# thomwiggers/m4ri-rust

Measured on AMD Instinct MI355X. Metric: gf2_matmul_bit_ops_per_sec_n65536, higher is better.
Workload: dtype u64

## Files before the change

m4ri-rust_amd/csrc/gf2_kernels.h:

```cpp
#pragma once
#include <hip/hip_runtime.h>
#include <stdint.h>

struct gf2k_mul_args {
  const uint64_t *A;
  const uint64_t *B;
  uint64_t *C;
  long long lda, ldb, ldc;
  long long sA, sB, sC;
  int m, l, n;
  int tiles_m, tiles_n;
  int ksplit;
  int kwords;
  int batch;
  int accumulate;
  const uint32_t *Bp;
  long long sBp;
  int bp_nc;
  uint64_t *P;
  long long ldp, sP;
  int a_packed;
  int n_rem, nseg;
  long long p_words;
  int n_full, seg_slabs, tile_slabs;
// ... 8 lines not shown
  int scan;
  int lastword;
  unsigned long long pcmask;
  int cur_row[64];
  int cntP, cnt2;
  int err;
};
enum { GF2K_ELIM_BLOCK_PIVOTS = 2048 };

extern "C" {
hipError_t gf2k_elim_begin_block(gf2k_elim_state *st, hipStream_t s);
hipError_t gf2k_elim_step(uint64_t *A, long long lda, int m, long long c0w, int sw, int j, uint64_t colmask, int full,
                          uint64_t *U, long long ldu, int uw, gf2k_elim_state *st, int *pivcols, uint64_t *ptab,
                          unsigned char *rowflag, int *blkpiv, uint64_t colmask_next, int lookahead, hipStream_t s);
hipError_t gf2k_elim_end_block(uint64_t *A, long long lda, long long aw, long long c0w, uint64_t *U, long long ldu, int uw,
                               gf2k_elim_state *st, unsigned char *rowflag, const int *blkpiv, int *moves, uint64_t *tmp,
                               long long tld, long long w_right, hipStream_t s);
hipError_t gf2k_elim_small(uint64_t *A, long long lda, int m, int ncols, int limit, int full, int *rank_out, int *pivcols,
                           hipStream_t s);
enum {
  GF2K_ELIM_BATCH_WAVE1 = 0,
  GF2K_ELIM_BATCH_WAVE2 = 1,
  GF2K_ELIM_BATCH_WAVE4 = 2,
  GF2K_ELIM_BATCH_WAVE8 = 3,
  GF2K_ELIM_BATCH_WAVE16 = 4,
  GF2K_ELIM_BATCH_WAVE_INV = 5,
  GF2K_ELIM_BATCH_LDS = 6,
  GF2K_ELIM_BATCH_LDS_INV = 7,
  GF2K_ELIM_BATCH_VARIANTS = 8
};
enum { GF2K_ELIM_BATCH_WAVE_THREADS = 256 };
hipError_t gf2k_elim_batch(const uint64_t *S, long long lds_, uint64_t *D, long long ldd, int m, int ncols, int limit, int full,
                           int inverse, long long batch, int *ranks, int *pivcols, int *singular, hipStream_t s);
hipError_t gf2k_set_diag(uint64_t *M, long long ld, int n, long long col0, hipStream_t s);
hipError_t gf2k_scatter_rows(uint64_t *X, long long ldx, const uint64_t *R, long long ldr, int words, const int *pivcols,
                             int rank, hipStream_t s);
hipError_t gf2k_any_nonzero(const uint64_t *M, long long ld, int row_lo, int rows, int cols, int *flag, hipStream_t s);
int gf2k_m4rm_rows_per_tile(int cfg);
long long gf2k_m4rm_streamk_words(int cfg, int nseg);
int gf2k_m4rm_cols_per_tile(int cfg);
hipError_t gf2k_packA(uint64_t *dst, long long wp, const uint64_t *src, long long lds_, int m, int w, hipStream_t stream);
hipError_t gf2k_m4rm(gf2k_mul_args a, int cfg, hipStream_t stream);
#ifdef GF2K_DEV_VARIANTS
hipError_t gf2k_dbg_sec(unsigned long long *out8);
int gf2k_packB_chunks(int l);
hipError_t gf2k_packB(uint32_t *Bp, long long bpStride, const uint64_t *B, long long ldb, long long bStride, int l, int n,
                      int batch, hipStream_t stream);
#endif
hipError_t gf2k_rowparity(const uint64_t *A, long long lda, const uint64_t *Bt, long long ldbt, uint64_t *C, long long ldc,
                          int m, int l, int n, int accumulate, hipStream_t stream);
hipError_t gf2k_narrow(const uint64_t *A, long long lda, const uint64_t *B, long long ldb, uint64_t *C, long long ldc,
                       int m, int l, int n, int accumulate, hipStream_t stream);
hipError_t gf2k_widevec(const uint64_t *A, long long lda, const uint64_t *Bt, long long ldbt, uint64_t *C, long long ldc,
                        int m, int l, int n, int accumulate, int jshift, hipStream_t stream);
hipError_t gf2k_tallskinny(const uint64_t *A, long long lda, const uint64_t *B, long long ldb, uint64_t *C, long long ldc,
                           int m, int l, int n, int accumulate, hipStream_t stream);
hipError_t gf2k_tallskinny_side(const uint64_t *A, long long lda, const uint64_t *B, long long ldb, uint64_t *C, long long ldc, int m,
                                int l, int n, uint64_t *side, long long side_ld, hipStream_t stream);
hipError_t gf2k_tallskinny_long(const uint64_t *A, long long lda, const uint64_t *B, long long ldb, uint64_t *C, long long ldc,
                                int m, int l, int n, int accumulate, hipStream_t stream);
hipError_t gf2k_va(const uint64_t *A, long long lda, const uint64_t *B, long long ldb, uint64_t *C, long long ldc, int m,
                   int l, int n, hipStream_t stream);
hipError_t gf2k_xor2d(uint64_t *C, long long ldc, const uint64_t *A, long long lda, const uint64_t *B, long long ldb,
                      int rows, int words, hipStream_t stream);
hipError_t gf2k_padcopy(uint64_t *dst, long long ldd, int drows, int dwords, const uint64_t *src, long long lds_, int srows,
                        int scols, hipStream_t stream);
hipError_t gf2k_copy_block(uint64_t *D, long long ldd, long long dr, long long dc, const uint64_t *S, long long lds_, long long sr,
                           long long sc, int nrows, int ncols, int accumulate, int zero_tail, hipStream_t stream);
hipError_t gf2k_fill_random(uint64_t *M, long long ld, int rows, int cols, uint64_t seed, long long row0, long long fullw,
                            long long colw0, hipStream_t stream);
hipError_t gf2k_diff(const uint64_t *A, long long lda, const uint64_t *B, long long ldb, int rows, int cols, int *diff,
                     hipStream_t stream);
hipError_t gf2k_transpose(uint64_t *D, long long ldd, const uint64_t *S, long long lds_, int rows, int cols,
                          hipStream_t stream);
hipError_t gf2k_strassen_split(uint64_t *dst, long long ldd, long long dstStride, const uint64_t *src, long long lds_,
                               long long srcStride, int h, int w, int side, int batch, hipStream_t stream);
hipError_t gf2k_strassen_split2(uint64_t *dst, long long ldd, long long dstStride, const uint64_t *src, long long lds_,
                                long long srcStride, int h, int w, int side, int batch, hipStream_t stream);
hipError_t gf2k_strassen_split3(uint64_t *dst, long long ldd, long long dstStride, const uint64_t *const *src0,
                                const uint64_t *const *src1, int groups, long long lds_, long long srcStride, int h, int w, int side,
                                int batch, hipStream_t stream);
hipError_t gf2k_strassen_merge3(uint64_t *dst, long long ldd, long long dstStride, const uint64_t *src, long long lds_,
                                long long srcStride, int h, int w, int accumulate, int groups, int batch, hipStream_t stream);
hipError_t gf2k_strassen_merge2(uint64_t *dst, long long ldd, long long dstStride, const uint64_t *src, long long lds_,
                                long long srcStride, int h, int w, int accumulate, int batch, hipStream_t stream);
hipError_t gf2k_strassen_merge(uint64_t *dst, long long ldd, long long dstStride, const uint64_t *src, long long lds_,
                               long long srcStride, int h, int w, int accumulate, int batch, hipStream_t stream);
}

void gf2k_note_launch(const void *kernel);
#undef hipLaunchKernelGGL
#define hipLaunchKernelGGL(kernelName, ...)                        \
  do {                                                             \
    gf2k_note_launch(reinterpret_cast<const void *>(kernelName));  \
    hipLaunchKernelGGLInternal((kernelName), __VA_ARGS__);         \
  } while (0)
```

m4ri-rust_amd/csrc/gf2_kernels.hip:

```cpp
#include <hip/hip_runtime.h>
#include <stdint.h>
#include <stdio.h>
#include <stdlib.h>
#include <algorithm>
#include <mutex>
#include <set>
#include <type_traits>
#include <utility>
#include "gf2_kernels.h"
#include "gf2_variants.h"

typedef uint64_t u64;
typedef uint32_t u32;

#ifdef GF2K_DEV_VARIANTS
#define GF2K_DEV_ENV(name, dflt) (getenv(name) ? atoi(getenv(name)) : (dflt))
__device__ unsigned long long *gf2k_clock_stamps;
extern "C" hipError_t gf2k_dev_set_clock_stamps(unsigned long long *p) {
  return hipMemcpyToSymbol(HIP_SYMBOL(gf2k_clock_stamps), &p, sizeof(p));
}
#else
#define GF2K_DEV_ENV(name, dflt) (dflt)
#endif

// ... 1964 lines not shown
      constexpr int a1 = kStrassenSupp[SIDE][q1][0], b1 = kStrassenSupp[SIDE][q1][1];
      u64 y[16];
      static_for<16>([&](auto J) {
        constexpr int j = decltype(J)::value;
        y[j] = b1 >= 0 ? (x[a1 * 16 + j] ^ x[(b1 < 0 ? 0 : b1) * 16 + j]) : x[a1 * 16 + j];
      });
      static_for<7>([&](auto Q2) {
        constexpr int q2 = decltype(Q2)::value;
        constexpr int a2 = kStrassenSupp[SIDE][q2][0], b2 = kStrassenSupp[SIDE][q2][1];
        u64 z[4];
        static_for<4>([&](auto J) {
          constexpr int j = decltype(J)::value;
          z[j] = b2 >= 0 ? (y[a2 * 4 + j] ^ y[(b2 < 0 ? 0 : b2) * 4 + j]) : y[a2 * 4 + j];
        });
        static_for<7>([&](auto Q3) {
          constexpr int q3 = decltype(Q3)::value;
          constexpr int a3 = kStrassenSupp[SIDE][q3][0], b3 = kStrassenSupp[SIDE][q3][1];
          const u64 o = b3 >= 0 ? (z[a3] ^ z[b3 < 0 ? 0 : b3]) : z[a3];
          if (NT) __builtin_nontemporal_store(o, &Y[(long long)(49 * q1 + 7 * q2 + q3) * dstStride + at]);
          else Y[(long long)(49 * q1 + 7 * q2 + q3) * dstStride + at] = o;
        });
      });
    });
  }
}

__device__ constexpr int kStrassenFoldTo[7][2] = {{0, 3}, {2, 3}, {1, 3}, {0, 2}, {0, 1}, {3, -1}, {0, -1}};

template <bool NT>
__global__ __launch_bounds__(256) void gf2_strassen_merge3_kernel(u64 *__restrict__ dst, long long ldd, long long dstStride,
                                                                  const u64 *__restrict__ src, long long lds_,
                                                                  long long srcStride, int h, int w, int accumulate) {
  const long long parent = (long long)blockIdx.z * gridDim.y + blockIdx.y;
  const u64 *M = src + parent * 343 * srcStride;
  u64 *Cq = dst + parent * dstStride;
  const long long total = (long long)h * w;
  for (long long idx = (long long)blockIdx.x * blockDim.x + threadIdx.x; idx < total; idx += (long long)gridDim.x * blockDim.x) {
    const int r = (int)(idx / w), c = (int)(idx % w);
    const u64 *Mp = M + (long long)r * lds_ + c;
    u64 z[64];
    static_for<64>([&](auto K) { z[decltype(K)::value] = 0; });
#pragma unroll 1
    for (int q1 = 0; q1 < 7; ++q1) {
      u64 y[16];
      static_for<16>([&](auto J) { y[decltype(J)::value] = 0; });
      const u64 *Mq = Mp + (long long)(49 * q1) * srcStride;
      static_for<7>([&](auto Q2) {
        constexpr int q2 = decltype(Q2)::value;
        u64 m[7];
        static_for<7>([&](auto Q3) {
          constexpr int q3 = decltype(Q3)::value;
          m[q3] = NT ? __builtin_nontemporal_load(&Mq[(long long)(7 * q2 + q3) * srcStride]) : Mq[(long long)(7 * q2 + q3) * srcStride];
        });
        const u64 f[4] = {m[0] ^ m[3] ^ m[4] ^ m[6], m[2] ^ m[4], m[1] ^ m[3], m[0] ^ m[1] ^ m[2] ^ m[5]};
        constexpr int t0 = kStrassenFoldTo[q2][0], t1 = kStrassenFoldTo[q2][1];
        static_for<4>([&](auto J) {
          constexpr int j = decltype(J)::value;
          y[t0 * 4 + j] ^= f[j];
          if (t1 >= 0) y[(t1 < 0 ? 0 : t1) * 4 + j] ^= f[j];
        });
      });
      const int u0 = kStrassenFoldTo[q1][0], u1 = kStrassenFoldTo[q1][1];
      static_for<4>([&](auto U) {
        constexpr int u = decltype(U)::value;
        const u64 mask = (u == u0 || u == u1) ? ~0ull : 0ull;
        static_for<16>([&](auto J) {
          constexpr int j = decltype(J)::value;
          z[u * 16 + j] ^= y[j] & mask;
        });
      });
    }
    static_for<64>([&](auto K) {
      constexpr int k = decltype(K)::value;
      constexpr int R = 4 * ((k >> 5) & 1) + 2 * ((k >> 3) & 1) + ((k >> 1) & 1);
      constexpr int Cc = 4 * ((k >> 4) & 1) + 2 * ((k >> 2) & 1) + (k & 1);
      u64 *pd = Cq + (long long)(r + R * h) * ldd + (long long)Cc * w + c;
      u64 v = z[k];
      if (accumulate) v ^= *pd;
      if (NT) __builtin_nontemporal_store(v, pd);
      else *pd = v;
    });
  }
}


static inline int grid_for(long long total, int block = 256, int cap = 256 * 8) {
  long long g = (total + block - 1) / block;
  if (g < 1) g = 1;
  if (g > cap) g = cap;
  return (int)g;
}

static int cfg_v8_rg(int cfg) { return gf2_variant_of(cfg).v8_rg; }
static int cfg_v9_rg(int cfg) { return gf2_variant_of(cfg).v9_rg; }
extern "C" int gf2k_m4rm_rows_per_tile(int cfg) { return gf2_variant_of(cfg).rows; }
extern "C" int gf2k_m4rm_cols_per_tile(int cfg) { return gf2_variant_of(cfg).cols; }
extern "C" long long gf2k_m4rm_streamk_words(int cfg, int nseg) { return gf2_streamk_words(gf2_variant_of(cfg), nseg); }

static hipError_t lds_limit_once(const void *kernel, int bytes) {
  static std::mutex mu;
  static std::set<std::pair<const void *, int>> done;
  int dev = 0;
  if (hipGetDevice(&dev) != hipSuccess) dev = 0;
  std::lock_guard<std::mutex> lk(mu);
  if (done.count({kernel, dev})) return hipSuccess;
  const hipError_t e = hipFuncSetAttribute(kernel, hipFuncAttributeMaxDynamicSharedMemorySize, bytes);
  if (e == hipSuccess) done.insert({kernel, dev});
  return e;
}

template <typename K>
static hipError_t launch_tile_kernel(K kernel, int threads, const gf2k_mul_args &a, long long nwg, hipStream_t stream) {
  hipError_t e = lds_limit_once(reinterpret_cast<const void *>(kernel), kLdsBytes);
  if (e != hipSuccess) {
    fprintf(stderr, "gf2k: hipFuncSetAttribute failed: %s\n", hipGetErrorString(e));
    return e;
  }
  hipLaunchKernelGGL(kernel, dim3((unsigned)nwg), dim3(threads), kLdsBytes, stream, a);
  e = hipGetLastError();
  if (e != hipSuccess) fprintf(stderr, "gf2k: tile kernel launch failed: %s\n", hipGetErrorString(e));
  return e;
}

static hipError_t launch_v8(gf2k_mul_args a, int cfg, int RG, hipStream_t stream) {
  const bool v9 = cfg_v9_rg(cfg) != 0;
  const int R = 512 * RG, TC = v9 ? 128 : 512;
  a.tiles_m = (a.m + R - 1) / R;
  a.tiles_n = (a.n + TC - 1) / TC;
  const long long T = (long long)a.tiles_m * a.tiles_n * a.batch;
  if (T > 0x7fffff00LL) return hipErrorInvalidValue;
  const int nw32 = (a.l + 31) / 32, Q = v9 ? (nw32 + 3) / 4 : (nw32 + 1) / 2;
  a.tile_slabs = Q;
  if (a.ksplit > 1 && a.n_rem <= 0) a.n_rem = (int)T, a.nseg = (int)std::min<long long>(T * a.ksplit, 1 << 20);
  a.ksplit = 1;
  a.kwords = 0;
#ifdef GF2K_DEV_VARIANTS
  static const int v8_flags = getenv("GF2K_V8_FLAGS") ? atoi(getenv("GF2K_V8_FLAGS")) : 0;
  a.kwords = v8_flags;
#endif
  long long n_rem = a.P && Q > 0 ? std::min<long long>(std::max(a.n_rem, 0), T) : 0;
  gf2_streamk_cut cut = gf2_streamk_cut_of(T, Q, n_rem, a.nseg);
  if (cut.nseg > 0x7fffff00LL - T || gf2_streamk_words(gf2_variant_of(cfg), cut.nseg) > a.p_words) cut = {0, 0, 0};
  n_rem = cut.n_rem;
  const int nseg = (int)cut.nseg, seg = (int)cut.seg;
  a.n_rem = (int)n_rem;
  a.nseg = nseg;
  a.seg_slabs = seg;
  a.n_full = (int)(T - n_rem);
  a.sP = (long long)R * (v9 ? 2 : 8);
  const long long nwg = (long long)a.n_full + nseg;
  if (nwg <= 0) return hipSuccess;
  hipError_t e = hipErrorInvalidValue;
#define GF2K_V8G(RGv, Gv)                                                                              \
  e = a.a_packed ? launch_tile_kernel(&gf2_m4rm_kernel_v8<RGv, Gv, 1>, 512, a, nwg, stream)            \
                 : launch_tile_kernel(&gf2_m4rm_kernel_v8<RGv, Gv, 0>, 512, a, nwg, stream)
#define GF2K_V8(RGv) GF2K_V8G(RGv, 2)
#define GF2K_V9(RGv)                                                                                   \
  e = a.a_packed ? launch_tile_kernel(&gf2_m4rm_kernel_v9<RGv, 2, 1>, 512, a, nwg, stream)             \
                 : launch_tile_kernel(&gf2_m4rm_kernel_v9<RGv, 2, 0>, 512, a, nwg, stream)
#ifdef GF2K_DEV_VARIANTS
  if (v9) {
    switch (RG) {
      case 8: GF2K_V9(8); break;
      case 4: GF2K_V9(4); break;
      default: GF2K_V9(2); break;
    }
// ... 545 lines not shown
    const long long ntp = (long long)((tx_n + stw - 1) / stw) * ((ty_n + 7) / 8) * (stw * 8);
    if (ntp > 0x7fffffffLL) return hipErrorInvalidValue;
    static const int tgrid = GF2K_DEV_ENV("M4RI_HIP_TRANSPOSE_GRID", (1 << 20));
    dim3 grid((unsigned)std::min<long long>(ntp, tgrid)), block(512);
    hipLaunchKernelGGL(gf2_transpose512_kernel, grid, block, 0, stream, D, ldd, S, lds_, rows, cols, (int)ntp, tflags);
    return hipGetLastError();
  }
  dim3 grid((sw + 3) / 4, rb), block(256);
  hipLaunchKernelGGL(gf2_transpose_kernel, grid, block, 0, stream, D, ldd, S, lds_, rows, cols);
  return hipGetLastError();
}

extern "C" hipError_t gf2k_strassen_split(u64 *dst, long long ldd, long long dstStride, const u64 *src, long long lds_,
                                          long long srcStride, int h, int w, int side, int batch, hipStream_t stream) {
  if (h <= 0 || w <= 0 || batch <= 0) return hipSuccess;
  const long long total = (long long)h * (w / 2);
  int gx = grid_for(total, 256, (4096 + batch - 1) / batch);
  hipLaunchKernelGGL(gf2_strassen_split_kernel, dim3(gx, 1, batch), dim3(256), 0, stream, dst, ldd, dstStride, src, lds_,
                     srcStride, h, w, side);
  return hipGetLastError();
}

extern "C" hipError_t gf2k_strassen_split2(u64 *dst, long long ldd, long long dstStride, const u64 *src, long long lds_,
                                           long long srcStride, int h, int w, int side, int batch, hipStream_t stream) {
  if (h <= 0 || w <= 0 || batch <= 0) return hipSuccess;
  const long long total = (long long)h * (w / 2);
  int gx = grid_for(total, 256, (4096 + batch - 1) / batch);
  hipLaunchKernelGGL(gf2_strassen_split2_kernel, dim3(gx, 1, batch), dim3(256), 0, stream, dst, ldd, dstStride, src, lds_,
                     srcStride, h, w, side);
  return hipGetLastError();
}

extern "C" hipError_t gf2k_strassen_split3(u64 *dst, long long ldd, long long dstStride, const u64 *const *src0,
                                           const u64 *const *src1, int groups, long long lds_, long long srcStride, int h, int w,
                                           int side, int batch, hipStream_t stream) {
  if (h <= 0 || w <= 0 || batch <= 0 || groups <= 0) return hipSuccess;
  if (groups > 7 || (side == 2 && (h & 63))) return hipErrorInvalidValue;
  gf2k_split3_srcs srcs{};
  for (int g = 0; g < groups; ++g) {
    srcs.a[g] = src0[g];
    srcs.b[g] = src1 ? src1[g] : nullptr;
  }
  const long long total = (long long)h * w;
  static const int cap = GF2K_DEV_ENV("M4RI_HIP_PASS_GRID", 8192);
  const int gx = grid_for(total, 256, (cap + batch * groups - 1) / (batch * groups));
  const dim3 grid(gx * groups, 1, batch);
  static const int nt = GF2K_DEV_ENV("M4RI_HIP_PASS_NT", 1);
#ifdef GF2K_DEV_VARIANTS
  if (!nt && side == 2)
    hipLaunchKernelGGL((gf2_strassen_split3_kernel<0, true>), grid, dim3(256), 0, stream, dst, ldd, dstStride, srcs, lds_, srcStride, h, w, gx);
  else if (!nt && side == 1)
    hipLaunchKernelGGL((gf2_strassen_split3_kernel<1, false>), grid, dim3(256), 0, stream, dst, ldd, dstStride, srcs, lds_, srcStride, h, w, gx);
  else
#endif
  if (side == 2)
    hipLaunchKernelGGL((gf2_strassen_split3_kernel<0, true, true>), grid, dim3(256), 0, stream, dst, ldd, dstStride, srcs, lds_, srcStride, h, w, gx);
  else if (side == 0)
    hipLaunchKernelGGL((gf2_strassen_split3_kernel<0, false>), grid, dim3(256), 0, stream, dst, ldd, dstStride, srcs, lds_, srcStride, h, w, gx);
  else
    hipLaunchKernelGGL((gf2_strassen_split3_kernel<1, false, true>), grid, dim3(256), 0, stream, dst, ldd, dstStride, srcs, lds_, srcStride, h, w, gx);
  (void)nt;
  return hipGetLastError();
}

extern "C" hipError_t gf2k_strassen_merge3(u64 *dst, long long ldd, long long dstStride, const u64 *src, long long lds_,
                                           long long srcStride, int h, int w, int accumulate, int groups, int batch,
                                           hipStream_t stream) {
  if (h <= 0 || w <= 0 || batch <= 0 || groups <= 0) return hipSuccess;
  const long long total = (long long)h * w;
  const int gx = grid_for(total, 256, (8192 + batch * groups - 1) / (batch * groups));
  static const int ntl = GF2K_DEV_ENV("M4RI_HIP_PASS_NTL", 1);
#ifdef GF2K_DEV_VARIANTS
  if (!ntl)
    hipLaunchKernelGGL(gf2_strassen_merge3_kernel<false>, dim3(gx, groups, batch), dim3(256), 0, stream, dst, ldd, dstStride, src, lds_,
                       srcStride, h, w, accumulate);
  else
#endif
    hipLaunchKernelGGL(gf2_strassen_merge3_kernel<true>, dim3(gx, groups, batch), dim3(256), 0, stream, dst, ldd, dstStride, src, lds_,
                       srcStride, h, w, accumulate);
  (void)ntl;
  return hipGetLastError();
}

extern "C" hipError_t gf2k_strassen_merge2(u64 *dst, long long ldd, long long dstStride, const u64 *src, long long lds_,
                                           long long srcStride, int h, int w, int accumulate, int batch,
                                           hipStream_t stream) {
  if (h <= 0 || w <= 0 || batch <= 0) return hipSuccess;
  const long long total = (long long)h * (w / 2);
  int gx = grid_for(total, 256, (4096 + batch - 1) / batch);
  hipLaunchKernelGGL(gf2_strassen_merge2_kernel, dim3(gx, 1, batch), dim3(256), 0, stream, dst, ldd, dstStride, src, lds_,
                     srcStride, h, w, accumulate);
  return hipGetLastError();
}

extern "C" hipError_t gf2k_strassen_merge(u64 *dst, long long ldd, long long dstStride, const u64 *src, long long lds_,
                                          long long srcStride, int h, int w, int accumulate, int batch,
                                          hipStream_t stream) {
  if (h <= 0 || w <= 0 || batch <= 0) return hipSuccess;
  const long long total = (long long)h * (w / 2);
  int gx = grid_for(total, 256, (4096 + batch - 1) / batch);
  hipLaunchKernelGGL(gf2_strassen_merge_kernel, dim3(gx, 1, batch), dim3(256), 0, stream, dst, ldd, dstStride, src, lds_,
                     srcStride, h, w, accumulate);
  return hipGetLastError();
}
```

m4ri-rust_amd/csrc/mul_dev_host.cpp:

```cpp
#include <algorithm>
#include <cstdint>
#include <vector>

#include "dev_args.h"
#include "gf2_kernels.h"
#include "mul_plan.h"

typedef uint64_t u64;

static int sync_if(bool sync_free, hipStream_t s) {
  return sync_free && hipStreamSynchronize(s) != hipSuccess ? gf2_fail_hip(hipGetLastError(), "hipStreamSynchronize") : 0;
}
static int launch_m4rm(gf2k_mul_args a, int cfg, hipStream_t s) {
  HIP_TRY(gf2k_m4rm(a, cfg, s));
  return 0;
}

static int apply_tile_plan(gf2k_mul_args &a, const TilePlan &tp, hipStream_t s) {
  a.ksplit = 1;
  a.n_rem = a.nseg = 0;
  a.P = nullptr;
  a.p_words = 0;
  const size_t want = tp.scratch();
  if (want == 0) return 0;
// ... 162 lines not shown
  const std::vector<PlanStep> plan = strassen_plan(L);
  u64 *Aop[7], *Bop[7], *Pop[7];
  auto at = [&](size_t off) { return off == StrassenArena::none ? nullptr : static_cast<u64 *>(ws) + off; };
  for (int i = 0; i < 7; ++i) Aop[i] = at(arena.a[i]), Bop[i] = at(arena.b[i]), Pop[i] = at(arena.p[i]);
  bool a_packed = false;
  const TilePlan leaf = leaf_plan(m, l, n, L, &a_packed);

  auto split_step = [&](const PlanStep &st, int prev, int i, int side, bool pack) -> int {
    const bool isA = side == 0;
    const int rows_prev = (isA ? m : l) >> prev, rows_i = (isA ? m : l) >> i;
    const int words_prev = ((isA ? l : n) >> prev) / 64, words_i = ((isA ? l : n) >> i) / 64;
    const int batch = (int)pow7(prev);
    const gf2_dmat *top = isA ? A : B;
    const u64 *src = prev ? (isA ? Aop[prev] : Bop[prev]) : top->data;
    const long long lds_ = prev ? (long long)words_prev : top->ld;
    const long long srcStride = prev ? (long long)rows_prev * lds_ : 0;
    u64 *dst = isA ? Aop[i] : Bop[i];
    const long long dstStride = (long long)rows_i * words_i;
    const int kside = pack ? 2 : side;
    if (st.k == 1) return (int)gf2k_strassen_split(dst, words_i, dstStride, src, lds_, srcStride, rows_i, words_i, kside, batch, s);
    if (st.k == 2) return (int)gf2k_strassen_split2(dst, words_i, dstStride, src, lds_, srcStride, rows_i, words_i, kside, batch, s);
    const u64 *s0[7], *s1[7];
    int groups = 1;
    s0[0] = src;
    s1[0] = nullptr;
    if (st.virt) {
      groups = 7;
      const long long hq = rows_prev / 2, wq = words_prev / 2;
      auto quad = [&](int q) { return src + (long long)(q >> 1) * hq * lds_ + (long long)(q & 1) * wq; };
      for (int g = 0; g < 7; ++g) {
        s0[g] = quad(kSupp[side][g][0]);
        s1[g] = kSupp[side][g][1] >= 0 ? quad(kSupp[side][g][1]) : nullptr;
      }
    }
    return (int)gf2k_strassen_split3(dst, words_i, dstStride, s0, s1, groups, lds_, srcStride, rows_i, words_i, kside, batch, s);
  };

  auto run = [&]() -> int {
    int prev = 0;
    for (size_t k = 0; k < plan.size(); ++k) {
      const int i = prev + plan[k].levels();
      const bool last = k + 1 == plan.size();
      HIP_TRY((hipError_t)split_step(plan[k], prev, i, 0, last && a_packed));
      HIP_TRY((hipError_t)split_step(plan[k], prev, i, 1, false));
      prev = i;
    }
    {
      const int mL = m >> L, lL = l >> L, nL = n >> L;
      gf2k_mul_args a{};
      a.lda = lL / 64;
      a.ldb = nL / 64;
      a.ldc = nL / 64;
      a.sA = (long long)mL * a.lda;
      a.sB = (long long)lL * a.ldb;
      a.sC = (long long)mL * a.ldc;
      a.A = Aop[L];
      a.B = Bop[L];
      a.C = Pop[L];
      a.m = mL;
      a.l = lL;
      a.n = nL;
      a.batch = (int)pow7(L);
      a.accumulate = 0;
      a.a_packed = a_packed ? 1 : 0;
      if (int r = launch_planned(a, leaf, s)) return r;
    }
    int i = L;
    for (int k = (int)plan.size() - 1; k >= 0; --k) {
      const PlanStep &st = plan[k];
      const int up = i - st.levels();
      const int mi = m >> i, wi = (n >> i) / 64, batch = (int)pow7(up);
      u64 *dst = up ? Pop[up] : C->data;
      const long long ldd = up ? (long long)((n >> up) / 64) : C->ld;
      const long long strD = up ? (long long)(m >> up) * ldd : 0;
      const int acc = up ? 0 : accumulate;
      const long long dP = (long long)mi * wi;
      if (st.k == 1) {
        HIP_TRY(gf2k_strassen_merge(dst, ldd, strD, Pop[i], wi, dP, mi, wi, acc, batch, s));
      } else if (st.k == 2) {
        HIP_TRY(gf2k_strassen_merge2(dst, ldd, strD, Pop[i], wi, dP, mi, wi, acc, batch, s));
      } else if (!st.virt) {
        HIP_TRY(gf2k_strassen_merge3(dst, ldd, strD, Pop[i], wi, dP, mi, wi, acc, 1, batch, s));
      } else {
        const int m1 = m >> (up + 1), w1 = (n >> (up + 1)) / 64;
        HIP_TRY(gf2k_strassen_merge3(Pop[up + 1], w1, (long long)m1 * w1, Pop[i], wi, dP, mi, wi, 0, 7, batch, s));
        HIP_TRY(gf2k_strassen_merge(dst, ldd, strD, Pop[up + 1], w1, (long long)m1 * w1, m1, w1, acc, batch, s));
      }
      i = up;
    }
    return 0;
  };
  const int rc = run();
  return rc ? rc : sync_if(sync_free, s);
}

static int cap_levels_by_memory(int m, int l, int n, int L, hipStream_t s, size_t extra_bytes = 0) {
  if (L <= 0) return L;
  const size_t avail = gf2_dev_arena_limit(s);
  while (L > 0 && strassen_arena(m, l, n, L).words * sizeof(u64) + extra_bytes > avail) --L;
  return L;
}

std::mutex gf2_enqueue_mu;

static int mul_strassen_padded(gf2_dmat *C, const gf2_dmat *A, const gf2_dmat *B, int accumulate, const MulPlan &pp, hipStream_t s) {
  const int m = A->nrows, l = A->ncols, n = B->ncols;
  const int mp = pp.d[0], lp = pp.d[1], np = pp.d[2];
  const long long wa = lp / 64, wb = np / 64;
  const size_t wordsA = (size_t)mp * wa, wordsB = (size_t)lp * wb, wordsC = (size_t)mp * wb;
  void *ws = nullptr;
  if (int rc = gf2_stream_scratch(s, (wordsA + wordsB + wordsC) * sizeof(u64), &ws, GF2_SLOT_PADDED)) return rc;
  u64 *pa = static_cast<u64 *>(ws), *pb = pa + wordsA, *pc = pb + wordsB;
  HIP_TRY(gf2k_padcopy(pa, wa, mp, (int)wa, A->data, A->ld, m, l, s));
  HIP_TRY(gf2k_padcopy(pb, wb, lp, (int)wb, B->data, B->ld, l, n, s));
  gf2_dmat Ap{pa, wa, mp, lp}, Bp{pb, wb, lp, np}, Cp{pc, wb, mp, np};
  if (int rc = mul_strassen(&Cp, &Ap, &Bp, 0, pp.L, s, false)) return rc;
  HIP_TRY(gf2k_xor2d(C->data, C->ld, pc, wb, accumulate ? C->data : nullptr, C->ld, m, words_of(n), s));
  return 0;
}

static int mul_strassen_peeled(gf2_dmat *C, const gf2_dmat *A, const gf2_dmat *B, int accumulate, const MulPlan &pp, hipStream_t s) {
  const int m = A->nrows, l = A->ncols, n = B->ncols;
  const int mc = pp.d[0], lc = pp.d[1], nc = pp.d[2];
  gf2_dmat Ac{A->data, A->ld, mc, lc}, Bc{B->data, B->ld, lc, nc}, Cc{C->data, C->ld, mc, nc};
  if (int rc = mul_strassen(&Cc, &Ac, &Bc, accumulate, pp.L, s, false)) return rc;
  auto strip = [&](gf2_dmat *Cs, const gf2_dmat *As, const gf2_dmat *Bs, int acc) -> int {
    int Ls = pick_levels(As->nrows, As->ncols, Bs->ncols, 0, strassen_leaf_min());
    Ls = cap_levels_by_memory(As->nrows, As->ncols, Bs->ncols, Ls, s);
    return mul_strassen(Cs, As, Bs, acc, Ls, s, false);
  };
  if (l > lc) {
    gf2_dmat At{A->data + lc / 64, A->ld, mc, l - lc}, Bt{B->data + (long long)lc * B->ld, B->ld, l - lc, nc};
    if (int rc = strip(&Cc, &At, &Bt, 1)) return rc;
  }
  if (n > nc) {
    gf2_dmat Ar{A->data, A->ld, mc, l}, Br{B->data + nc / 64, B->ld, l, n - nc}, Cr{C->data + nc / 64, C->ld, mc, n - nc};
    if (int rc = strip(&Cr, &Ar, &Br, accumulate)) return rc;
  }
  if (m > mc) {
    gf2_dmat Ab{A->data + (long long)mc * A->ld, A->ld, m - mc, l}, Cb{C->data + (long long)mc * C->ld, C->ld, m - mc, n};
    if (int rc = strip(&Cb, &Ab, B, accumulate)) return rc;
  }
  return 0;
}

static int mul_naive_dev(gf2_dmat *C, const gf2_dmat *A, const gf2_dmat *B, int accumulate, hipStream_t s,
                         bool sync_free) {
  const int m = A->nrows, l = A->ncols, n = B->ncols;
  if (n > 64 || l == 0) return gf2_mul_m4rm_plain(C, A, B, accumulate, s);
  if (m == 0 || n == 0) return 0;
  if (ts_long_shape(m, l, n)) {
    HIP_TRY(gf2k_tallskinny_long(A->data, A->ld, B->data, B->ld, C->data, C->ld, m, l, n, accumulate, s));
    return sync_if(sync_free, s);
  }
  if (widevec_shape(m, l, n)) {
    if (int rc = mul_widevec(C, A, B, accumulate, s)) return rc;
    return sync_if(sync_free, s);
  }
  if (n > 8 && m >= 2048) return gf2_mul_m4rm_plain(C, A, B, accumulate, s);
  static const int narrow_lpn_rows = dev_env_int("M4RI_HIP_NARROW_LPN_ROWS", 262144);
  if (narrow_lpn_rows > 0 && m >= narrow_lpn_rows && l <= 256 && l > 64) {
    HIP_TRY(gf2k_tallskinny(A->data, A->ld, B->data, B->ld, C->data, C->ld, m, l, n, accumulate, s));
    return sync_if(sync_free, s);
  }
  if ((size_t)n * words_of(l) * 8 <= 65536) {
    hipError_t e1 = gf2k_narrow(A->data, A->ld, B->data, B->ld, C->data, C->ld, m, l, n, accumulate, s);
    if (e1 != hipSuccess) return gf2_fail_hip(e1, "gf2k_narrow");
    return sync_if(sync_free, s);
  }
// ... 145 lines not shown
```

m4ri-rust_amd/csrc/mul_plan_host.cpp:

```cpp
#include <array>
#include <cmath>
#include <cstdio>
#include <unordered_map>

#include "../../include/m4ri_hip.h"
#include "mul_plan.h"

typedef uint64_t u64;

int strassen_leaf_min() {
  static const int leaf_min = env_int("M4RI_HIP_STRASSEN_LEAF_MIN", 2048);
  return leaf_min;
}

struct TileGeom {
  int rows, cols;
  double cyc_per_chunk;
};
static TileGeom tile_geom(int cfg, bool packed = false) {
  const gf2_variant v = gf2_variant_of(cfg);
  return {v.rows, v.cols, v.cols == 512 ? (packed ? 1520.0 : 1800.0) : v.cols == 1024 ? (packed ? 1620.0 : 1790.0) : v.rows == 256 ? 1300.0 : 2350.0};
}
static long long tiles_of(const TileGeom &g, int m, int n) {
  return (long long)((m + g.rows - 1) / g.rows) * ((n + g.cols - 1) / g.cols);
// ... 215 lines not shown
      head.band_rows = m2;
      head.band = {band.cfg, band.n_rem, band.nseg, band.ws_bytes};
      consider(head);
    }
  }
  if (!have && v8_model(m, l, n, batch, packed, 12, 0, 0, c)) consider(c);
  return best;
}

static const double kPackLaunch = 5.0e-6;
PlainPlan plain_plan(int m, int l, int n) {
  static const double bw = (double)dev_env_int("M4RI_HIP_STREAM_GBS", 5000) * 1e9;
  static const int plain_pack = env_int("M4RI_HIP_PLAIN_APACK", 1);
  PlainPlan pp{plan_tiles(m, l, n, 1, false), false, 0.0};
  pp.t = pp.tp.t;
  const long long wp = (words_of(l) + 1) & ~1ll, prow = ((long long)m + 63) & ~63ll;
  if (plain_pack && m >= 512 && prow * wp * 8 < (1ll << 32)) {
    const TilePlan pk = plan_tiles(m, l, n, 1, true);
    const double t = pk.t + 2.0 * (double)prow * (double)wp * 8.0 / bw + kPackLaunch;
    if (cfg_reads_packed(pk.cfg) && t < pp.t) pp = {pk, true, t};
  }
  return pp;
}
static double plain_time_model(int m, int l, int n) { return plain_plan(m, l, n).t; }

std::vector<PlanStep> strassen_plan(int L) {
  const int fuse3 = env_int("M4RI_HIP_STRASSEN_FUSE3", 1);
  std::vector<PlanStep> p;
  if (L <= 0) return p;
  if (!fuse3) {
    if (L & 1) p.push_back({1, false});
    for (int lv = L & 1; lv < L; lv += 2) p.push_back({2, false});
    return p;
  }
  switch (L) {
    case 1: p = {{1, false}}; break;
    case 2: p = {{2, false}}; break;
    case 3: p = {{3, false}}; break;
    case 4: p = {{3, true}}; break;
    case 5: p = {{2, false}, {3, false}}; break;
    default: p = {{3, false}, {3, false}}; break;
  }
  return p;
}

static bool strassen_packs_a(int m, int L) {
  static const int apack_on = env_int("M4RI_HIP_APACK", 1);
  if (!apack_on || L < 1) return false;
  return ((m >> L) & 63) == 0;
}

size_t pow7(int i) {
  size_t p = 1;
  while (i-- > 0) p *= 7;
  return p;
}

TilePlan leaf_plan(int m, int l, int n, int L, bool *a_packed) {
  const int batch = (int)pow7(L);
  TilePlan tp = plan_tiles(m >> L, l >> L, n >> L, batch, false);
  bool packed = false;
  if (strassen_packs_a(m, L)) {
    const TilePlan pk = plan_tiles(m >> L, l >> L, n >> L, batch, true);
    if (cfg_reads_packed(pk.cfg) && pk.t <= tp.t) tp = pk, packed = true;
  }
  if (a_packed) *a_packed = packed;
  return tp;
}
static double leaf_time_model(int m, int l, int n, int L) {
  const double t = leaf_plan(m, l, n, L).t;
  return strassen_packs_a(m, L) ? std::min(t, plan_tiles(m >> L, l >> L, n >> L, (int)pow7(L), true).t) : t;
}

static double strassen_pass_bytes(double m, double l, double n, int L) {
  double bytes = 0;
  int prev = 0;
  for (const PlanStep &st : strassen_plan(L)) {
    const int i = prev + st.levels();
    const double p7 = (double)pow7(prev);
    const double a_i = (m * l) / std::pow(4.0, i) / 8.0, b_i = (l * n) / std::pow(4.0, i) / 8.0, c_i = (m * n) / std::pow(4.0, i) / 8.0;
    const double rd = st.virt ? 12.0 * std::pow(4.0, st.k) : std::pow(4.0, st.k), wr = std::pow(7.0, st.levels());
    bytes += p7 * (rd + wr) * (a_i + b_i);
    if (st.virt)
      bytes += p7 * c_i * (wr + 7.0 * std::pow(4.0, st.k) + 7.0 * std::pow(4.0, st.k) + std::pow(4.0, st.k + 1));
    else
      bytes += p7 * c_i * (wr + std::pow(4.0, st.k));
    prev = i;
  }
  return bytes;
}

static const double kPassLaunch = 5.0e-6;
static double level_time_model(int m, int l, int n, int L) {
  static const double bw = (double)dev_env_int("M4RI_HIP_STREAM_GBS", 5000) * 1e9;
  if (L <= 0) return plain_time_model(m, l, n);
  const int d = 1 << L;
  if (L > 6 || m % d || l % (128 * d) || n % (128 * d)) return -1.0;
  return leaf_time_model(m, l, n, L) + strassen_pass_bytes(m, l, n, L) / bw +
         3 * kPassLaunch * (double)strassen_plan(L).size();
}
extern "C" double gf2_model_time(int m, int l, int n, int levels) { return level_time_model(m, l, n, levels); }

static int pick_levels_uncached(int m, int l, int n, int req, int leaf_min, double *t_out);
int pick_levels(int m, int l, int n, int req, int leaf_min, double *t_out) {
  struct Res {
    int L;
    double t;
  };
  thread_local std::unordered_map<PlanKey, Res, PlanKeyHash> memo;
  const PlanKey key{m, l, n, req, leaf_min * 2 + (env_int("M4RI_HIP_STRASSEN_FUSE3", 1) ? 1 : 0)};
  const Res res = memoised(memo, key, [&] {
    Res r{0, 0.0};
    r.L = pick_levels_uncached(m, l, n, req, leaf_min, &r.t);
    return r;
  });
  if (t_out) *t_out = res.t;
  return res.L;
}
static int pick_levels_uncached(int m, int l, int n, int req, int leaf_min, double *t_out) {
  static const int max_auto = std::min(env_int("M4RI_HIP_STRASSEN_MAX_LEVELS", 5), 6);
  const int cap = req > 0 ? (req > 6 ? 6 : req) : max_auto;
  int best = 0;
  double best_t = 0;
  for (int L = 0; L <= cap; ++L) {
    if (L > 0) {
      const int d = 1 << L;
      if (m % d || l % (128 * d) || n % (128 * d)) break;
      if (req <= 0 && ((m >> L) < (leaf_min < 1024 ? leaf_min : 1024) || (l >> L) < leaf_min || (n >> L) < leaf_min)) break;
    }
    if (req > 0) {
      best = L;
      continue;
    }
    double t = level_time_model(m, l, n, L);
    if (L == 0 || t < best_t * (L >= 3 ? 0.97 : 0.985)) {
      best = L;
      best_t = t;
    }
  }
  if (t_out) *t_out = best_t;
  return best;
}

StrassenArena strassen_arena(int m, int l, int n, int L) {
  StrassenArena ar;
  std::fill_n(ar.a, 7, ar.none), std::fill_n(ar.b, 7, ar.none), std::fill_n(ar.p, 7, ar.none);
  if (L > 6) L = 6;
  int prev = 0;
  for (const PlanStep &st : strassen_plan(L)) {
    const int i = prev + st.levels();
    const size_t mi = (size_t)m >> i, li = (size_t)l >> i, ni = (size_t)n >> i, p7 = pow7(i);
    ar.a[i] = ar.words;
    ar.words += p7 * mi * (li / 64);
    ar.b[i] = ar.words;
    ar.words += p7 * li * (ni / 64);
    ar.p[i] = ar.words;
    ar.words += p7 * mi * (ni / 64);
    if (st.virt) {
      ar.p[prev + 1] = ar.words;
      ar.words += pow7(prev + 1) * ((size_t)m >> (prev + 1)) * (((size_t)n >> (prev + 1)) / 64);
    }
    prev = i;
  }
  return ar;
}

bool widevec_shape(int m, int l, int n) {
// ... 294 lines not shown
```

Before: 19410000 billion.

## Fuse virtual four-level Strassen merge into a single LDS-accumulating kernel

Replaces the two-pass virtual merge (merge3 into a temporary, then merge) with a new merge4 kernel. It folds all 7^4 products per output element in registers and LDS using atomic XORs, then writes the 256 output blocks directly. The aim is to drop the intermediate temporary's write and re-read traffic, plus one launch, and the planner's byte model is updated to match. In exchange it uses heavy register arrays (64+16 u64 per thread), 128KB of LDS, and LDS atomics, which may limit occupancy.

```diff
diff --git a/m4ri-rust_amd/csrc/gf2_kernels.h b/m4ri-rust_amd/csrc/gf2_kernels.h
--- a/m4ri-rust_amd/csrc/gf2_kernels.h
+++ b/m4ri-rust_amd/csrc/gf2_kernels.h
@@ -114,6 +114,8 @@
                                 int batch, hipStream_t stream);
 hipError_t gf2k_strassen_merge3(uint64_t *dst, long long ldd, long long dstStride, const uint64_t *src, long long lds_,
                                 long long srcStride, int h, int w, int accumulate, int groups, int batch, hipStream_t stream);
+hipError_t gf2k_strassen_merge4(uint64_t *dst, long long ldd, long long dstStride, const uint64_t *src, long long lds_,
+                                long long srcStride, int h, int w, int accumulate, int batch, hipStream_t stream);
 hipError_t gf2k_strassen_merge2(uint64_t *dst, long long ldd, long long dstStride, const uint64_t *src, long long lds_,
                                 long long srcStride, int h, int w, int accumulate, int batch, hipStream_t stream);
 hipError_t gf2k_strassen_merge(uint64_t *dst, long long ldd, long long dstStride, const uint64_t *src, long long lds_,
diff --git a/m4ri-rust_amd/csrc/gf2_kernels.hip b/m4ri-rust_amd/csrc/gf2_kernels.hip
--- a/m4ri-rust_amd/csrc/gf2_kernels.hip
+++ b/m4ri-rust_amd/csrc/gf2_kernels.hip
@@ -2070,6 +2070,8 @@
     });
   }
 }
+
+#include "strassen/gf2_merge4.inc"
 
 
 static inline int grid_for(long long total, int block = 256, int cap = 256 * 8) {
@@ -2781,6 +2783,17 @@
   return hipGetLastError();
 }
 
+extern "C" hipError_t gf2k_strassen_merge4(u64 *dst, long long ldd, long long dstStride, const u64 *src, long long lds_,
+                                           long long srcStride, int h, int w, int accumulate, int batch, hipStream_t stream) {
+  if (h <= 0 || w <= 0 || batch <= 0) return hipSuccess;
+  const hipError_t e = lds_limit_once(reinterpret_cast<const void *>(&gf2_strassen_merge4_kernel), kMerge4LdsBytes);
+  if (e != hipSuccess) return e;
+  const int gx = grid_for((long long)h * w, 64, (256 + batch - 1) / batch);
+  hipLaunchKernelGGL(gf2_strassen_merge4_kernel, dim3(gx, batch), dim3(kMerge4Threads), kMerge4LdsBytes, stream, dst, ldd, dstStride,
+                     src, lds_, srcStride, h, w, accumulate);
+  return hipGetLastError();
+}
+
 extern "C" hipError_t gf2k_strassen_merge2(u64 *dst, long long ldd, long long dstStride, const u64 *src, long long lds_,
                                            long long srcStride, int h, int w, int accumulate, int batch,
                                            hipStream_t stream) {
diff --git a/m4ri-rust_amd/csrc/mul_dev_host.cpp b/m4ri-rust_amd/csrc/mul_dev_host.cpp
--- a/m4ri-rust_amd/csrc/mul_dev_host.cpp
+++ b/m4ri-rust_amd/csrc/mul_dev_host.cpp
@@ -268,9 +268,7 @@
       } else if (!st.virt) {
         HIP_TRY(gf2k_strassen_merge3(dst, ldd, strD, Pop[i], wi, dP, mi, wi, acc, 1, batch, s));
       } else {
-        const int m1 = m >> (up + 1), w1 = (n >> (up + 1)) / 64;
-        HIP_TRY(gf2k_strassen_merge3(Pop[up + 1], w1, (long long)m1 * w1, Pop[i], wi, dP, mi, wi, 0, 7, batch, s));
-        HIP_TRY(gf2k_strassen_merge(dst, ldd, strD, Pop[up + 1], w1, (long long)m1 * w1, m1, w1, acc, batch, s));
+        HIP_TRY(gf2k_strassen_merge4(dst, ldd, strD, Pop[i], wi, dP, mi, wi, acc, batch, s));
       }
       i = up;
     }
diff --git a/m4ri-rust_amd/csrc/mul_plan_host.cpp b/m4ri-rust_amd/csrc/mul_plan_host.cpp
--- a/m4ri-rust_amd/csrc/mul_plan_host.cpp
+++ b/m4ri-rust_amd/csrc/mul_plan_host.cpp
@@ -321,7 +321,7 @@
     const double rd = st.virt ? 12.0 * std::pow(4.0, st.k) : std::pow(4.0, st.k), wr = std::pow(7.0, st.levels());
     bytes += p7 * (rd + wr) * (a_i + b_i);
     if (st.virt)
-      bytes += p7 * c_i * (wr + 7.0 * std::pow(4.0, st.k) + 7.0 * std::pow(4.0, st.k) + std::pow(4.0, st.k + 1));
+      bytes += p7 * c_i * (wr + std::pow(4.0, st.k + 1));
     else
       bytes += p7 * c_i * (wr + std::pow(4.0, st.k));
     prev = i;
diff --git a/m4ri-rust_amd/csrc/strassen/gf2_merge4.inc b/m4ri-rust_amd/csrc/strassen/gf2_merge4.inc
--- /dev/null
+++ b/m4ri-rust_amd/csrc/strassen/gf2_merge4.inc
@@ -0,0 +1,80 @@
+
+constexpr int kMerge4Waves = 7;
+constexpr int kMerge4Threads = kMerge4Waves * 64;
+constexpr int kMerge4LdsBytes = 4 * 64 * 64 * 8;
+
+__global__ __launch_bounds__(kMerge4Threads) void gf2_strassen_merge4_kernel(u64 *__restrict__ dst, long long ldd, long long dstStride,
+                                                                             const u64 *__restrict__ src, long long lds_,
+                                                                             long long srcStride, int h, int w, int accumulate) {
+  extern __shared__ u64 merge4_sums[];
+  const int lane = threadIdx.x & 63, q0 = threadIdx.x >> 6;
+  const u64 *M = src + ((long long)blockIdx.y * 7 + q0) * 343 * srcStride;
+  u64 *Cq = dst + (long long)blockIdx.y * dstStride;
+  const long long total = (long long)h * w, nblocks = (total + 63) >> 6;
+  for (int i = threadIdx.x; i < 4 * 64 * 64; i += kMerge4Threads) merge4_sums[i] = 0;
+  __syncthreads();
+  for (long long blk = blockIdx.x; blk < nblocks; blk += gridDim.x) {
+    const long long idx = blk * 64 + lane;
+    const bool live = idx < total;
+    const int r = (int)(idx / w), c = (int)(idx % w);
+    if (live) {
+      const u64 *Mp = M + (long long)r * lds_ + c;
+      u64 z[64];
+      static_for<64>([&](auto K) { z[decltype(K)::value] = 0; });
+#pragma unroll 1
+      for (int q1 = 0; q1 < 7; ++q1) {
+        u64 y[16];
+        static_for<16>([&](auto J) { y[decltype(J)::value] = 0; });
+        const u64 *Mq = Mp + (long long)(49 * q1) * srcStride;
+        static_for<7>([&](auto Q2) {
+          constexpr int q2 = decltype(Q2)::value;
+          u64 m[7];
+          static_for<7>([&](auto Q3) {
+            constexpr int q3 = decltype(Q3)::value;
+            m[q3] = __builtin_nontemporal_load(&Mq[(long long)(7 * q2 + q3) * srcStride]);
+          });
+          const u64 f[4] = {m[0] ^ m[3] ^ m[4] ^ m[6], m[2] ^ m[4], m[1] ^ m[3], m[0] ^ m[1] ^ m[2] ^ m[5]};
+          constexpr int t0 = kStrassenFoldTo[q2][0], t1 = kStrassenFoldTo[q2][1];
+          static_for<4>([&](auto J) {
+            constexpr int j = decltype(J)::value;
+            y[t0 * 4 + j] ^= f[j];
+            if (t1 >= 0) y[(t1 < 0 ? 0 : t1) * 4 + j] ^= f[j];
+          });
+        });
+        const int u0 = kStrassenFoldTo[q1][0], u1 = kStrassenFoldTo[q1][1];
+        static_for<4>([&](auto U) {
+          constexpr int u = decltype(U)::value;
+          const u64 mask = (u == u0 || u == u1) ? ~0ull : 0ull;
+          static_for<16>([&](auto J) {
+            constexpr int j = decltype(J)::value;
+            z[u * 16 + j] ^= y[j] & mask;
+          });
+        });
+      }
+      const int v0 = kStrassenFoldTo[q0][0], v1 = kStrassenFoldTo[q0][1];
+      unsigned long long *s0 = reinterpret_cast<unsigned long long *>(merge4_sums) + v0 * 4096 + lane;
+      static_for<64>([&](auto K) { atomicXor(s0 + decltype(K)::value * 64, z[decltype(K)::value]); });
+      if (v1 >= 0) {
+        unsigned long long *s1 = reinterpret_cast<unsigned long long *>(merge4_sums) + v1 * 4096 + lane;
+        static_for<64>([&](auto K) { atomicXor(s1 + decltype(K)::value * 64, z[decltype(K)::value]); });
+      }
+    }
+    __syncthreads();
+    for (int j0 = q0 * 8; j0 < 256; j0 += kMerge4Waves * 8) {
+      u64 v[8];
+      u64 *pd[8];
+      static_for<8>([&](auto I) {
+        constexpr int i = decltype(I)::value;
+        const int j = j0 + i, qd = j >> 6;
+        const int R = 8 * (qd >> 1) + 4 * ((j >> 5) & 1) + 2 * ((j >> 3) & 1) + ((j >> 1) & 1);
+        const int Cc = 8 * (qd & 1) + 4 * ((j >> 4) & 1) + 2 * ((j >> 2) & 1) + (j & 1);
+        pd[i] = Cq + (long long)(r + R * h) * ldd + (long long)Cc * w + c;
+        v[i] = merge4_sums[j * 64 + lane];
+        merge4_sums[j * 64 + lane] = 0;
+        if (accumulate && live) v[i] ^= *pd[i];
+      });
+      if (live) static_for<8>([&](auto I) { __builtin_nontemporal_store(v[decltype(I)::value], pd[decltype(I)::value]); });
+    }
+    __syncthreads();
+  }
+}
```

Result: faster. 19690000 billion, median of 6 (+1.4%).
